# talmolab/VNL-Brax-Imitation

Hardware: AMD Instinct MI355X
Metric: env-steps/sec (whole node), rodent imitation, num_envs=4096/GPU (higher is better)
Workload: dtype f32; 1 GPU; rodent imitation rollout, single groom clip, 4096 envs/GPU: intention-policy forward (HIP) -> RodentTracking.step (5 substeps, CG 6/6) -> auto-reset on -> Transition logging (unroll 20, the 20 steps replayed as one captured hipGraph); envs_per_gpu=4096, clips=1, parallelism=env-sharded x1, no data-path collective

## Files before the change

### include/vnl.h

```cpp
#ifndef VNL_H_
#define VNL_H_

#include <stddef.h>
#include <stdint.h>

#ifdef __cplusplus
extern "C" {
#endif

#define VNL_OK 0
#define VNL_ERR_ARG -1
#define VNL_ERR_BLOB -2
#define VNL_ERR_HIP -3
#define VNL_ERR_NO_DEVICE -4
#define VNL_ERR_UNSUPPORTED -5

typedef struct vnl_model vnl_model;
typedef struct vnl_env vnl_env;
typedef struct vnl_policy vnl_policy;

typedef struct vnl_envspec {
  int32_t clip_frames;
  int32_t num_clips;
  int32_t ref_traj_length;
// ... 125 lines not shown
                       const float* rand_action ,
                       float* rand_log_prob ,
                       void* stream);

typedef struct vnl_policy_noise {
  uint64_t seed;
  const int64_t* step_base;
  int64_t step_offset;
  int64_t env_offset;
  float *eps_latent_out, *eps_action_out, *rand_action_out;
} vnl_policy_noise;
int vnl_policy_forward_noise(vnl_policy*, const float* params, const float* obs_mean, const float* obs_std,
                             const float* traj, const float* obs, const vnl_policy_noise*, int32_t batch,
                             int32_t deterministic, float* action, float* raw_action, float* log_prob, float* logits,
                             float* latent_mean, float* latent_logvar, float* rand_log_prob , void* stream);

#define VNL_POST_MAX_OPS 24
typedef struct vnl_post_op {
  float* dst;
  const float* src;
  const float* first;
  float* log;
  int32_t width;
  int32_t pad_;
} vnl_post_op;
typedef struct vnl_post_desc {
  float *steps, *prev_done, *done, *truncation;
  const float* reward;
  float *log_reward, *log_discount, *log_truncation;
  int32_t episode_length, action_repeat, num_ops, pad_;
  vnl_post_op ops[VNL_POST_MAX_OPS];
} vnl_post_desc;
int vnl_rollout_post(const vnl_post_desc*, int32_t num_envs, void* stream);

typedef struct vnl_ppo_head_args {
  int32_t T, B, act, latent;
  const float *logits, *baseline, *bootstrap, *lat_mean, *lat_logvar;
  const float *raw_action, *behaviour_log_prob, *reward, *truncation, *discount, *eps_entropy;
  float entropy_cost, discounting, reward_scaling, gae_lambda, clipping_epsilon, kl_weight, min_std, var_scale;
  int32_t normalize_advantage, pad_;
  float *g_logits, *g_baseline, *g_lat_mean, *g_lat_logvar;
  float *vs, *advantages;
  float *metrics;
} vnl_ppo_head_args;
#define VNL_PPO_HEAD_WORKSPACE_FLOATS (4 + 4 * 256)
int vnl_ppo_head(const vnl_ppo_head_args*, float* workspace, void* stream);

typedef struct vnl_gather_op {
  float* dst;
  const float* src;
  int32_t T, width;
} vnl_gather_op;
typedef struct vnl_gather_desc {
  const int64_t* idx;
  int32_t N, M, num_ops, pad_;
  vnl_gather_op ops[VNL_POST_MAX_OPS];
} vnl_gather_desc;
int vnl_gather_rows(const vnl_gather_desc*, void* stream);

int vnl_adam_step(float* params, const float* grads, float* mu, float* nu, const int64_t* count, int64_t n,
                  double lr, double b1, double b2, double eps, void* stream);

typedef struct vnl_ppo_net_spec {
  int32_t traj_size, obs_size, action_size, latent_size;
  int32_t num_encoder_layers, num_decoder_layers , num_value_layers ;
  int32_t encoder_layers[8], decoder_layers[8], value_layers[8];
// ... 38 lines not shown
```

### vnl-brax-imitation_amd/_lib.py

```python
from __future__ import annotations

import ctypes as C
import os

_HERE = os.path.dirname(os.path.abspath(__file__))
DEFAULT_LIB = os.path.join(_HERE, "csrc", "libvnl.so")

i32p = C.POINTER(C.c_int32)
f32p = C.POINTER(C.c_float)


class EnvSpec(C.Structure):
    _fields_ = [
        ("clip_frames", C.c_int32),
        ("num_clips", C.c_int32),
        ("ref_traj_length", C.c_int32),
        ("sub_clip_length", C.c_int32),
        ("n_frames", C.c_int32),
        ("num_track_bodies", C.c_int32),
        ("num_end_eff", C.c_int32),
        ("num_appendages", C.c_int32),
        ("num_joint_cols", C.c_int32),
        ("com_ref_col", C.c_int32),
        ("body_idxs", i32p),
# ... 106 lines not shown

PPO_HEAD_WORKSPACE_FLOATS = 4 + 4 * 256


class PPONetSpec(C.Structure):
    _fields_ = [(n, C.c_int32) for n in ("traj_size", "obs_size", "action_size", "latent_size", "num_encoder_layers",
                                          "num_decoder_layers", "num_value_layers")] + \
               [("encoder_layers", C.c_int32 * 8), ("decoder_layers", C.c_int32 * 8), ("value_layers", C.c_int32 * 8)]


class PPOBatch(C.Structure):
    _fields_ = [(n, C.c_void_p) for n in ("traj", "obs", "next_obs_last", "raw_action", "behaviour_log_prob", "reward",
                                          "truncation", "discount", "eps_latent", "eps_entropy", "obs_mean", "obs_std")]


class PPOHParams(C.Structure):
    _fields_ = [(n, C.c_float) for n in ("entropy_cost", "discounting", "reward_scaling", "gae_lambda",
                                         "clipping_epsilon", "kl_weight", "min_std", "var_scale")] + \
               [("normalize_advantage", C.c_int32), ("pad_", C.c_int32)]

class CorrPlan(C.Structure):
    _fields_ = [(n, C.c_int32) for n in ("route", "chunks", "chunk_cols", "row_tiles")] + [("workspace_floats", C.c_int64)]


class Domain(C.Structure):
    _fields_ = [(n, C.c_void_p) for n in ("cg_friction", "act_gain", "dof_damping", "dof_armature")]

class BodyDomain(C.Structure):
    _fields_ = [(n, C.c_void_p) for n in ("body_mass", "body_inertia", "body_ipos")]


EXPORTS = (
    "vnl_last_error", "vnl_version", "vnl_model_create", "vnl_model_destroy", "vnl_env_create", "vnl_env_destroy",
    "vnl_env_dims", "vnl_env_reset", "vnl_env_reset_done", "vnl_env_step", "vnl_env_fk", "vnl_env_debug", "vnl_env_scratch", "vnl_policy_create", "vnl_policy_destroy",
    "vnl_policy_num_params", "vnl_policy_forward", "vnl_policy_forward_noise", "vnl_rollout_post", "vnl_ppo_head", "vnl_adam_step", "vnl_gather_rows",
    "vnl_ppo_update_create", "vnl_ppo_update_destroy", "vnl_ppo_update_num_params", "vnl_ppo_update_buffer",
    "vnl_ppo_minibatch_grad",
    "vnl_ppo_minibatch_grad_part",
    "vnl_env_set_domain", "vnl_env_set_body_domain",
    "vnl_prediction_corr_plan", "vnl_prediction_corr",
)
_HIP_ONLY = ("vnl_policy_", "vnl_ppo_update_", "vnl_ppo_minibatch_", "vnl_prediction_corr")


class VnlError(RuntimeError):
    pass


def _declare(lib: C.CDLL) -> C.CDLL:
    vp = C.c_void_p
    lib.vnl_last_error.restype = C.c_char_p
    lib.vnl_version.restype = C.c_int
    lib.vnl_model_create.argtypes = [vp, C.c_size_t, C.POINTER(vp)]
    lib.vnl_model_destroy.argtypes = [vp]
    lib.vnl_model_destroy.restype = None
    lib.vnl_env_create.argtypes = [vp, C.POINTER(EnvSpec), C.c_int32, C.c_int32, C.POINTER(vp)]
    lib.vnl_env_destroy.argtypes = [vp]
    lib.vnl_env_destroy.restype = None
    lib.vnl_env_dims.argtypes = [vp, C.POINTER(Dims)]
    lib.vnl_env_reset.argtypes = [vp, vp, vp, C.POINTER(StatePtrs), vp]
    lib.vnl_env_reset_done.argtypes = [vp, vp, C.POINTER(ResetNoise), C.POINTER(StatePtrs), C.POINTER(ResetLog), C.c_int32, vp]
    lib.vnl_env_step.argtypes = [vp, vp, C.POINTER(StatePtrs), vp]
    lib.vnl_env_fk.argtypes = [vp, vp, C.POINTER(StatePtrs), vp]
    lib.vnl_env_debug.argtypes = [vp, C.c_int32, C.POINTER(C.c_int32)]
    lib.vnl_env_scratch.argtypes = [vp, C.c_char_p, C.POINTER(vp), C.POINTER(C.c_int32)]
    lib.vnl_env_set_domain.argtypes = [vp, C.POINTER(Domain), vp]
    lib.vnl_env_set_body_domain.argtypes = [vp, C.POINTER(BodyDomain), vp]
    lib.vnl_rollout_post.argtypes = [C.POINTER(PostDesc), C.c_int32, vp]
    lib.vnl_ppo_head.argtypes = [C.POINTER(PPOHeadArgs), vp, vp]
    lib.vnl_gather_rows.argtypes = [C.POINTER(GatherDesc), vp]
    lib.vnl_adam_step.argtypes = [vp, vp, vp, vp, vp, C.c_int64] + [C.c_double] * 4 + [vp]
    if hasattr(lib, "vnl_ppo_update_create"):
        lib.vnl_ppo_update_create.argtypes = [C.POINTER(PPONetSpec), C.c_int32, C.c_int32, C.c_int32, C.POINTER(vp)]
        lib.vnl_ppo_update_destroy.argtypes = [vp]
        lib.vnl_ppo_update_destroy.restype = None
        lib.vnl_ppo_update_num_params.argtypes = [vp]
        lib.vnl_ppo_update_num_params.restype = C.c_int64
        lib.vnl_ppo_update_buffer.argtypes = [vp, C.c_char_p, C.POINTER(vp), C.POINTER(C.c_int64)]
        lib.vnl_ppo_minibatch_grad.argtypes = [vp, vp, C.POINTER(PPOBatch), C.POINTER(PPOHParams), vp, vp, vp]
        lib.vnl_ppo_minibatch_grad_part.argtypes = [vp, vp, C.POINTER(PPOBatch), C.POINTER(PPOHParams), vp, vp, vp, C.c_int]
        lib.vnl_prediction_corr_plan.argtypes = [C.c_int32, C.c_int32, C.c_int32, C.POINTER(CorrPlan)]
        lib.vnl_prediction_corr.argtypes = [vp, vp, C.c_float, C.c_int32, C.c_int32, C.c_int32, vp, C.c_int64, vp, vp]
    if hasattr(lib, "vnl_policy_create"):
        lib.vnl_policy_create.argtypes = [C.POINTER(PolicySpec), C.c_int32, C.c_int32, C.POINTER(vp)]
        lib.vnl_policy_destroy.argtypes = [vp]
        lib.vnl_policy_destroy.restype = None
        lib.vnl_policy_num_params.argtypes = [vp]
        lib.vnl_policy_num_params.restype = C.c_int64
        lib.vnl_policy_forward.argtypes = [vp] + [vp] * 7 + [C.c_int32, C.c_int32] + [vp] * 6 + [vp, vp] + [vp]
        lib.vnl_policy_forward_noise.argtypes = [vp] + [vp] * 5 + [C.POINTER(PolicyNoise), C.c_int32, C.c_int32] + [vp] * 7 + [vp]
    return lib


_cache = {}

# ... 20 lines not shown
```

### vnl-brax-imitation_amd/csrc/vnl_domain.hip

```cpp
#include <hip/hip_runtime.h>
#include <stdint.h>

#include "../../include/vnl.h"
#ifdef VNL_PROFILE
#define g_vnl_prof g_vnl_prof_domain
#endif
#include "vnl_env_kernels.h"

int vnl_domain_reset_(const KernelConsts* kc, int spec, int B, size_t lds, void* stream, const DevState& ds, const int* start_frame,
                      const vreal* noise, vreal* dump, int* trace) {
  if (spec)
    hipLaunchKernelGGL((vnl_reset_kernel<VnlSpecDom<VnlSpecRodent>>), dim3(B), dim3(64), lds, (hipStream_t)stream, kc, ds,
                       start_frame, noise, dump, trace);
  else
    hipLaunchKernelGGL((vnl_reset_kernel<VnlSpecDom<VnlSpecGeneric>>), dim3(B), dim3(64), lds, (hipStream_t)stream, kc, ds,
                       start_frame, noise, dump, trace);
  return (int)hipGetLastError();
}

int vnl_domain_step_(const KernelConsts* kc, int spec, int B, size_t lds, void* stream, const DevState& ds, const vreal* action,
                     vreal* dump, vreal* dump_mid, int* trace) {
  if (spec)
    hipLaunchKernelGGL((vnl_step_kernel<VnlSpecDom<VnlSpecRodent>>), dim3(B), dim3(64), lds, (hipStream_t)stream, kc, ds,
                       action, dump, dump_mid, trace);
  else
    hipLaunchKernelGGL((vnl_step_kernel<VnlSpecDom<VnlSpecGeneric>>), dim3(B), dim3(64), lds, (hipStream_t)stream, kc, ds,
                       action, dump, dump_mid, trace);
  return (int)hipGetLastError();
}

int vnl_domain_reset_done_(const KernelConsts* kc, int spec, int B, size_t lds, void* stream, const DevState& ds,
                           const ResetDoneArgs& a, vreal* dump, int* trace) {
  if (spec)
    hipLaunchKernelGGL((vnl_reset_done_kernel<VnlSpecDom<VnlSpecRodent>>), dim3(B), dim3(64), lds, (hipStream_t)stream, kc, ds, a,
                       dump, trace);
  else
    hipLaunchKernelGGL((vnl_reset_done_kernel<VnlSpecDom<VnlSpecGeneric>>), dim3(B), dim3(64), lds, (hipStream_t)stream, kc, ds, a,
                       dump, trace);
  return (int)hipGetLastError();
}
```

### vnl-brax-imitation_amd/csrc/vnl_env_kernels.h

```cpp
#pragma once
#include "vnl_body.h"

#ifndef VNL_KERNEL_ATTR
#define VNL_KERNEL_ATTR
#endif
#define VNL_ENV_KERNEL __launch_bounds__(64) VNL_KERNEL_ATTR

template <class SP>
__global__ void VNL_ENV_KERNEL vnl_step_kernel(const KernelConsts* kc, DevState st, const vreal* action,
                                                      vreal* dump, vreal* dump_mid, int* trace) {
  VNL_LDS_DECL(lds);
  const VNL_CAS KernelConsts* k = VNL_TO_CAS(KernelConsts, kc);
  EnvWaveT<SP> w{k->m, k->ev, st, k->L, lds, blockIdx.x, threadIdx.x, k, nullptr};
  w.step(action, dump_mid, trace);
  if (dump) w.dump(dump);
}

template <class SP>
__global__ void VNL_ENV_KERNEL vnl_reset_kernel(const KernelConsts* kc, DevState st, const int* start_frame,
                                                       const vreal* noise, vreal* dump, int* trace) {
  VNL_LDS_DECL(lds);
  const VNL_CAS KernelConsts* k = VNL_TO_CAS(KernelConsts, kc);
  EnvWaveT<SP> w{k->m, k->ev, st, k->L, lds, blockIdx.x, threadIdx.x, k, nullptr};
  w.reset(start_frame, noise, trace);
  if (dump) w.dump(dump);
}


template <class SP>
__global__ void VNL_ENV_KERNEL vnl_reset_done_kernel(const KernelConsts* kc, DevState st, ResetDoneArgs a, vreal* dump, int* trace) {
  VNL_LDS_DECL(lds);
  const unsigned e = blockIdx.x, lane = threadIdx.x;
  if (a.mask[e] != 0.f) {
    const VNL_CAS KernelConsts* k = VNL_TO_CAS(KernelConsts, kc);
    EnvWaveT<SP> w{k->m, k->ev, st, k->L, lds, e, lane, k, nullptr};
    w.reset_fresh(a, trace);
    if (dump) w.dump(dump);
    VNL_SYNC_GLOBAL();
  }
  for (int q = 0; q < a.num_logs; q++) {
    const unsigned* src = a.logs[q].src + (size_t)e * a.logs[q].width;
    unsigned* log = a.logs[q].log + (size_t)e * a.logs[q].width;
    VNL_FOR(i, a.logs[q].width) log[i] = src[i];
  }
}
```

### vnl-brax-imitation_amd/csrc/vnl_lib.hip

```cpp
#include <hip/hip_runtime.h>
#include <stdint.h>
#include <stdio.h>
#include <stdlib.h>
#include <string.h>

#include <algorithm>
#include <cmath>
#include <cstddef>
#include <map>
#include <string>
#include <vector>

#include "../../include/vnl.h"
#include "vnl_body.h"

static thread_local char g_err[512] = "";
static int fail(int code, const char* fmt, const char* a = "", const char* b = "") {
  snprintf(g_err, sizeof(g_err), fmt, a, b);
  return code;
}
#define HIPCHK(call)                                                              \
  do {                                                                            \
    hipError_t e_ = (call);                                                       \
    if (e_ != hipSuccess) return fail(VNL_ERR_HIP, "%s: %s", #call, hipGetErrorString(e_)); \
// ... 958 lines not shown
  *count = it->second.second;
  return VNL_OK;
}

extern "C" int vnl_env_debug(vnl_env* env, int32_t enable, int32_t* row_stride) {
  if (!env) return fail(VNL_ERR_ARG, "vnl_env_debug: null argument");
  if (enable < 0 || enable > 2) return fail(VNL_ERR_ARG, "vnl_env_debug: mode must be 0, 1 or 2");
  if (enable && !env->dump) {
    void* p = nullptr;
    HIPCHK(hipMalloc(&p, (size_t)env->L.total * env->B * sizeof(vreal)));
    env->allocs.push_back(p);
    env->dump = (vreal*)p;
    const size_t nt = (size_t)env->B * (env->de.n_frames > 0 ? env->de.n_frames : 1) * VNL_TRACE_INTS * sizeof(int);
    HIPCHK(hipMalloc(&p, nt));
    env->allocs.push_back(p);
    HIPCHK(hipMemset(p, 0, nt));
    env->trace = (int*)p;
  }
  env->debug = enable;
  if (row_stride) *row_stride = env->L.total;
  return VNL_OK;
}

__global__ void __launch_bounds__(64) vnl_fk_kernel(const KernelConsts* kc, DevState st, const vreal* qpos) {
  VNL_LDS_DECL(lds);
  const VNL_CAS KernelConsts* k = VNL_TO_CAS(KernelConsts, kc);
  EnvWave w{k->m, k->ev, st, k->L, lds, blockIdx.x, threadIdx.x, k, nullptr};
  w.fk(qpos);
}

int vnl_domain_reset_(const KernelConsts* kc, int spec, int B, size_t lds, void* stream, const DevState& ds, const int* start_frame,
                      const vreal* noise, vreal* dump, int* trace);
int vnl_domain_step_(const KernelConsts* kc, int spec, int B, size_t lds, void* stream, const DevState& ds, const vreal* action,
                     vreal* dump, vreal* dump_mid, int* trace);
int vnl_domain_reset_done_(const KernelConsts* kc, int spec, int B, size_t lds, void* stream, const DevState& ds,
                           const ResetDoneArgs& a, vreal* dump, int* trace);

static int to_dev_state(const vnl_state* s, DevState* d) {
  const void* ptrs[] = {s->qpos, s->qvel, s->act, s->qacc_warmstart, s->xpos, s->xquat, s->subtree_com1,
                        s->qfrc_actuator, s->obs, s->reward, s->done, s->metrics, s->traj, s->termination_error,
                        s->cur_frame, s->sub_clip_frame, s->clip_id};
  for (const void* p : ptrs)
    if (!p) return fail(VNL_ERR_ARG, "vnl_state: null buffer");
  d->qpos = (vreal*)s->qpos, d->qvel = (vreal*)s->qvel, d->act = (vreal*)s->act, d->warm = (vreal*)s->qacc_warmstart;
  d->xpos = (vreal*)s->xpos, d->xquat = (vreal*)s->xquat, d->com1 = (vreal*)s->subtree_com1;
  d->qfrc_actuator = (vreal*)s->qfrc_actuator, d->obs = (vreal*)s->obs, d->reward = (vreal*)s->reward;
  d->done = (vreal*)s->done, d->metrics = (vreal*)s->metrics, d->traj = (vreal*)s->traj;
  d->term_err = (vreal*)s->termination_error, d->cur_frame = s->cur_frame, d->sub_clip_frame = s->sub_clip_frame;
  d->clip_id = s->clip_id;
  return VNL_OK;
}

extern "C" int vnl_env_reset(vnl_env* env, const int32_t* start_frame, const float* noise, const vnl_state* state,
                             void* stream) {
  if (!env || !start_frame || !noise || !state) return fail(VNL_ERR_ARG, "vnl_env_reset: null argument");
  DevState ds;
  int rc = to_dev_state(state, &ds);
  if (rc != VNL_OK) return rc;
  DeviceGuard guard(env->device);
  if (!guard.ok) return fail(VNL_ERR_HIP, "hipSetDevice failed");
  if (env->has_dom) {
    HIPCHK((hipError_t)vnl_domain_reset_(env->kc, env->spec, env->B, env->lds_bytes, stream, ds, (const int*)start_frame,
                                         (const vreal*)noise, env->debug ? env->dump : nullptr, env->debug ? env->trace : nullptr));
    return VNL_OK;
  }
  if (env->spec)
    hipLaunchKernelGGL((vnl_reset_kernel<VnlSpecRodent>), dim3(env->B), dim3(64), env->lds_bytes, (hipStream_t)stream,
// ... 33 lines not shown
  for (int k = 0; k < num_logs; k++)
    a.logs[k].src = (const unsigned*)logs[k].src, a.logs[k].log = (unsigned*)logs[k].log, a.logs[k].width = logs[k].width;
  DeviceGuard guard(env->device);
  if (!guard.ok) return fail(VNL_ERR_HIP, "hipSetDevice failed");
  vreal* dump = env->debug ? env->dump : nullptr;
  int* trace = env->debug ? env->trace : nullptr;
  if (env->has_dom) {
    HIPCHK((hipError_t)vnl_domain_reset_done_(env->kc, env->spec, env->B, env->lds_bytes, stream, ds, a, dump, trace));
    return VNL_OK;
  }
  if (env->spec)
    hipLaunchKernelGGL((vnl_reset_done_kernel<VnlSpecRodent>), dim3(env->B), dim3(64), env->lds_bytes, (hipStream_t)stream,
                       (const KernelConsts*)env->kc, ds, a, dump, trace);
  else
    hipLaunchKernelGGL((vnl_reset_done_kernel<VnlSpecGeneric>), dim3(env->B), dim3(64), env->lds_bytes, (hipStream_t)stream,
                       (const KernelConsts*)env->kc, ds, a, dump, trace);
  HIPCHK(hipGetLastError());
  return VNL_OK;
}

extern "C" int vnl_env_fk(vnl_env* env, const float* qpos, const vnl_state* state, void* stream) {
  if (!env || !qpos || !state) return fail(VNL_ERR_ARG, "vnl_env_fk: null argument");
  DevState ds;
  int rc = to_dev_state(state, &ds);
  if (rc != VNL_OK) return rc;
  DeviceGuard guard(env->device);
  if (!guard.ok) return fail(VNL_ERR_HIP, "hipSetDevice failed");
  hipLaunchKernelGGL(vnl_fk_kernel, dim3(env->B), dim3(64), env->lds_bytes, (hipStream_t)stream, (const KernelConsts*)env->kc, ds,
                     (const vreal*)qpos);
  HIPCHK(hipGetLastError());
  return VNL_OK;
}

extern "C" int vnl_env_step(vnl_env* env, const float* action, const vnl_state* state, void* stream) {
  if (!env || !action || !state) return fail(VNL_ERR_ARG, "vnl_env_step: null argument");
  DevState ds;
  int rc = to_dev_state(state, &ds);
  if (rc != VNL_OK) return rc;
  DeviceGuard guard(env->device);
  if (!guard.ok) return fail(VNL_ERR_HIP, "hipSetDevice failed");
  if (env->has_dom) {
    HIPCHK((hipError_t)vnl_domain_step_(env->kc, env->spec, env->B, env->lds_bytes, stream, ds, (const vreal*)action,
                                        env->debug == 1 ? env->dump : nullptr, env->debug == 2 ? env->dump : nullptr,
                                        env->debug ? env->trace : nullptr));
    return VNL_OK;
  }
  if (env->spec)
    hipLaunchKernelGGL((vnl_step_kernel<VnlSpecRodent>), dim3(env->B), dim3(64), env->lds_bytes, (hipStream_t)stream,
                       (const KernelConsts*)env->kc, ds, (const vreal*)action, env->debug == 1 ? env->dump : nullptr,
                       env->debug == 2 ? env->dump : nullptr, env->debug ? env->trace : nullptr);
  else
    hipLaunchKernelGGL((vnl_step_kernel<VnlSpecGeneric>), dim3(env->B), dim3(64), env->lds_bytes, (hipStream_t)stream,
                       (const KernelConsts*)env->kc, ds, (const vreal*)action, env->debug == 1 ? env->dump : nullptr,
                       env->debug == 2 ? env->dump : nullptr, env->debug ? env->trace : nullptr);
  HIPCHK(hipGetLastError());
  return VNL_OK;
}


static std::vector<vreal> four_field_tables(const vnl_env* env, const std::vector<double> v[4]) {
  const DevModel& d = env->dm;
  std::vector<vreal> tab;
  tab.reserve((size_t)env->B * (2 * d.ncg + d.nu + 2 * d.nv));
  for (double x : v[0]) tab.push_back((vreal)x);
  for (size_t k = 0; k < v[0].size(); k++) tab.push_back((vreal)contact_invweight(env->cg_t[k % d.ncg], v[0][k], env->impratio));
  for (int f = 1; f < 4; f++)
    for (double x : v[f]) tab.push_back((vreal)x);
  return tab;
}
static std::vector<vreal> four_field_compiled(const vnl_env* env) {
  const std::vector<double>* model[4] = {&env->mu0, &env->gain0, &env->damp0, &env->arm0};
  std::vector<double> v[4];
  for (int f = 0; f < 4; f++)
    for (int e = 0; e < env->B; e++) v[f].insert(v[f].end(), model[f]->begin(), model[f]->end());
  return four_field_tables(env, v);
}

static const char* body_row(const vnl_env* env, const double* mass, const double* inertia, const double* ipos, std::vector<double>* out,
                            char* why, size_t nwhy) {
  const int nb = env->fmap->nb_out, nd = env->dm.nbody;
  std::vector<double> full;
  if (inertia) {
    full = env->ifull0;
    for (int b = 1; b < nb; b++) {
      double dl[3], R[9];
      for (int k = 0; k < 3; k++) dl[k] = inertia[3 * (size_t)b + k] - env->inertia0[3 * (size_t)b + k];
      if (dl[0] == 0 && dl[1] == 0 && dl[2] == 0) continue;
      qmat_d(&env->iquat0[4 * (size_t)b], R);
      for (int r = 0; r < 3; r++)
// ... 207 lines not shown
  const unsigned e = blockIdx.x, tid = threadIdx.x;
  float st = d.steps ? ((d.prev_done && d.prev_done[e] != 0.f) ? 0.f : d.steps[e]) + (float)d.action_repeat : 0.f;
  float done = d.done[e];
  bool over = d.steps && st >= (float)d.episode_length;
  float trunc = over ? 1.f - done : 0.f;
  done = over ? 1.f : done;
  __syncthreads();
  if (tid == 0) {
    if (d.steps) d.steps[e] = st;
    if (d.prev_done) d.prev_done[e] = done;
    d.done[e] = done;
    if (d.truncation) d.truncation[e] = trunc;
    if (d.log_reward) d.log_reward[e] = d.reward[e];
    if (d.log_discount) d.log_discount[e] = 1.f - done;
    if (d.log_truncation) d.log_truncation[e] = trunc;
  }
  const bool reset = done != 0.f;
  for (int k = 0; k < d.num_ops; k++) {
    const vnl_post_op& op = d.ops[k];
    const bool from_first = op.first && reset;
    const unsigned* src = (const unsigned*)(from_first ? op.first : op.src) + (size_t)e * op.width;
    unsigned* dst = op.dst ? (unsigned*)op.dst + (size_t)e * op.width : nullptr;
    unsigned* log = op.log ? (unsigned*)op.log + (size_t)e * op.width : nullptr;
    const bool store = dst && (from_first || (const float*)op.dst != op.src);
    for (int i = (int)tid; i < op.width; i += VNL_POST_THREADS) {
      unsigned v = src[i];
      if (store) dst[i] = v;
      if (log) log[i] = v;
    }
  }
}

extern "C" int vnl_rollout_post(const vnl_post_desc* desc, int32_t num_envs, void* stream) {
  if (!desc || num_envs <= 0 || !desc->done) return fail(VNL_ERR_ARG, "vnl_rollout_post: null argument");
  if (desc->num_ops < 0 || desc->num_ops > VNL_POST_MAX_OPS) return fail(VNL_ERR_ARG, "vnl_rollout_post: too many ops");
  for (int k = 0; k < desc->num_ops; k++)
    if (!desc->ops[k].src || desc->ops[k].width <= 0) return fail(VNL_ERR_ARG, "vnl_rollout_post: bad op");
  if ((desc->log_reward && !desc->reward)) return fail(VNL_ERR_ARG, "vnl_rollout_post: log_reward without reward");
  hipLaunchKernelGGL(vnl_post_kernel, dim3(num_envs), dim3(VNL_POST_THREADS), 0, (hipStream_t)stream, *desc);
  HIPCHK(hipGetLastError());
  return VNL_OK;
}

#ifndef VNL_HEAD_THREADS
#define VNL_HEAD_THREADS 256
#define VNL_HEAD_GROUP 32
#define VNL_GROUP_SUM(v) \
  (v += __shfl_xor(v, 16, 32), v += __shfl_xor(v, 8, 32), v += __shfl_xor(v, 4, 32), v += __shfl_xor(v, 2, 32), v += __shfl_xor(v, 1, 32))
#endif
#define VNL_HEAD_MAXBLK 256
#ifndef VNL_FINISH_THREADS
#define VNL_FINISH_THREADS 64
#define VNL_FINISH_SUM(v) \
  (v += __shfl_xor(v, 32), v += __shfl_xor(v, 16), v += __shfl_xor(v, 8), v += __shfl_xor(v, 4), v += __shfl_xor(v, 2), v += __shfl_xor(v, 1))
#endif
__device__ __forceinline__ float vnl_block_sum(float v, float* red) {
  const unsigned tid = threadIdx.x;
  __syncthreads();
  red[tid] = v;
  __syncthreads();
  for (unsigned w = VNL_HEAD_THREADS / 2; w > 0; w >>= 1) {
    if (tid < w) red[tid] += red[tid + w];
    __syncthreads();
  }
  return red[0];
}
__device__ __forceinline__ float vnl_softplus(float x) { return x > 20.f ? x : log1pf(expf(x)); }

__global__ void __launch_bounds__(VNL_HEAD_THREADS) vnl_ppo_gae_kernel(vnl_ppo_head_args a, float* stats) {
#if VNL_HEAD_THREADS > 1
  __shared__ float red[VNL_HEAD_THREADS];
// ... 226 lines not shown
```

### vnl-brax-imitation_amd/envs/rodent.py

```python
from __future__ import annotations

import ctypes as C
import os
from typing import Any, Dict, List, Mapping, Optional, Sequence

import numpy as np
import torch

from .. import _lib
from ..model import blob as _blob
from ..model import mjcf as _mjcf
from .base import Env, PipelineState, State

_PKG = os.path.dirname(os.path.dirname(os.path.abspath(__file__)))
_TEST_BACKEND = None
_METRICS = ("rcom", "rvel", "rtrunk", "rquat", "ract", "rapp", "termination_error")
DOMAIN_FIELDS = {"cg_friction": ("ngeom_collide", 0.0, False), "act_gain": ("nu", None, False),
                 "dof_damping": ("nv", 0.0, True), "dof_armature": ("nv", 0.0, True)}
BODY_DOMAIN_FIELDS = {"body_mass": ((), 0.0), "body_inertia": ((3,), 0.0), "body_ipos": ((3,), None)}


def packaged_model_path(name: str = "rodent", scale_factor: Optional[float] = 0.9) -> str:
    if scale_factor is None:
        return os.path.join(_PKG, "data", f"{name}.npz")
# ... 335 lines not shown
        nz.start_hi = self._start_hi()
        nz.noise_scale = self._reset_noise_scale
        record = record or {}
        for k, dt in (("start_frame", torch.int32), ("clip_id", torch.int32), ("noise", self._dtype)):
            t = record.get(k)
            if t is not None:
                if t.dtype != dt or not t.is_contiguous() or t.shape[0] != B or t.device != self.device:
                    raise ValueError(f"record[{k!r}] must be a contiguous {dt} tensor with {B} rows on the env's device")
                setattr(nz, k + "_out", t.data_ptr())
        logs = tuple(logs)
        if len(logs) > _lib.RESET_MAX_LOGS:
            raise ValueError(f"at most {_lib.RESET_MAX_LOGS} logs")
        arr = (_lib.ResetLog * max(len(logs), 1))()
        for o, (src, log) in zip(arr, logs):
            if src.dtype not in (torch.float32, torch.int32) or log.dtype != src.dtype or src.shape != log.shape or \
                    src.shape[0] != B or not (src.is_contiguous() and log.is_contiguous()):
                raise ValueError("a log is a (src, log) pair of contiguous float32 / int32 tensors of one shape (B[, w])")
            o.src, o.log, o.width = src.data_ptr(), log.data_ptr(), src.numel() // B
        p = self._ptrs(state)
        _lib.check(self._L, self._L.vnl_env_reset_done(self._env_h, mk.data_ptr(), C.byref(nz), C.byref(p), arr, len(logs),
                                                       self._stream()))
        self._hold = (mk, step_base, logs, record)
        return state

    def step(self, state: State, action: torch.Tensor) -> State:
        nu, B = int(self.dims.nu), self.num_envs
        if tuple(action.shape) != (B, nu):
            raise ValueError(f"action must be ({B},{nu}), got {tuple(action.shape)}")
        a = action.to(device=self.device, dtype=self._dtype).contiguous()
        p = self._ptrs(state)
        ev = getattr(self, "kernel_events", None)
        if ev is not None:
            ev[0].record()
        _lib.check(self._L, self._L.vnl_env_step(self._env_h, a.data_ptr(), C.byref(p), self._stream()))
        if ev is not None:
            ev[1].record()
        self._hold = (a,)
        return state

    def forward_kinematics(self, qpos: torch.Tensor, out: Optional[State] = None) -> State:
        B, nq = self.num_envs, int(self.dims.nq)
        if tuple(qpos.shape) != (B, nq):
            raise ValueError(f"qpos must be ({B},{nq}), got {tuple(qpos.shape)}")
        state = out if out is not None else self._alloc_state()
        q = qpos.to(device=self.device, dtype=self._dtype).contiguous()
        state.pipeline_state.qpos.copy_(q)
        p = self._ptrs(state)
        _lib.check(self._L, self._L.vnl_env_fk(self._env_h, q.data_ptr(), C.byref(p), self._stream()))
        self._hold = (q,)
        return state

    def debug(self, mode=True) -> None:
        stride = C.c_int32()
        _lib.check(self._L, self._L.vnl_env_debug(self._env_h, int(mode), C.byref(stride)))
        self._dump_stride = stride.value

    def solver_trace(self) -> torch.Tensor:
        ptr, cnt = C.c_void_p(), C.c_int32()
        _lib.check(self._L, self._L.vnl_env_scratch(self._env_h, b"solver_trace", C.byref(ptr), C.byref(cnt)))
        B, n = self.num_envs, cnt.value
        if self.device.type == "cuda":
            torch.cuda.synchronize(self.device)
            flat = torch.empty(B * n, dtype=torch.int32, device=self.device)
            rc = C.CDLL("libamdhip64.so").hipMemcpy(C.c_void_p(flat.data_ptr()), ptr, C.c_size_t(4 * B * n), C.c_int(3))
            if rc != 0:
                raise _lib.VnlError(f"hipMemcpy failed: {rc}")
            flat = flat.cpu()
# ... 27 lines not shown
```

### vnl-brax-imitation_amd/ppo_imitation/acting.py

```python
from __future__ import annotations

import dataclasses
import time
from typing import Any, Callable, Dict, Optional, Sequence, Tuple

import numpy as np
import torch

from ..envs.base import State
from ..envs.wrappers import EvalWrapper


@dataclasses.dataclass
class Transition:

    observation: torch.Tensor
    action: torch.Tensor
    reward: torch.Tensor
    discount: torch.Tensor
    next_observation: torch.Tensor
    extras: Dict[str, Dict[str, torch.Tensor]]

    def map(self, fn: Callable[[torch.Tensor], torch.Tensor]) -> "Transition":
        return Transition(fn(self.observation), fn(self.action), fn(self.reward), fn(self.discount),
                          fn(self.next_observation),
                          {k: {kk: fn(vv) for kk, vv in v.items()} for k, v in self.extras.items()})


def actor_step(env, env_state: State, policy, key, extra_fields: Sequence[str] = ()) -> Tuple[State, Transition]:
    obs = env_state.obs.clone()
    traj = env_state.info["traj"]
    actions, policy_extras = policy(traj, obs, key)
    nstate = env.step(env_state, actions)
    state_extras = {x: nstate.info[x] for x in extra_fields}
    return nstate, Transition(observation=obs, action=actions, reward=nstate.reward, discount=1 - nstate.done,
                              next_observation=nstate.obs,
                              extras={"policy_extras": policy_extras, "state_extras": state_extras})


def _fusable(env):
    from ..envs import wrappers as W

    if not isinstance(env, W.AutoResetWrapper) or not isinstance(env.env, W.EpisodeWrapper):
        return None
    ep, base = env.env, env.env.env
    if ep.action_repeat != 1 or base is not base.unwrapped or not hasattr(getattr(base, "_L", None), "vnl_rollout_post"):
        return None
    return env, ep, base


def _device_noise(policy) -> bool:
    return getattr(policy, "noise", None) == "device"


_DIRECT_LOG = True


def _generate_unroll_fused(fz, env_state: State, policy, key, unroll_length: int, extra_fields) -> Tuple[State, Transition]:
    import ctypes as C

    from .. import _lib

    ar, ep, base = fz
    st = env_state
    T, info, dev = unroll_length, env_state.info, env_state.obs.device
    B = st.obs.shape[0]
    new = lambda *shape, like: torch.empty((T, *shape), dtype=like.dtype, device=dev)
    obs0, nobs_log = st.obs.clone(), new(*st.obs.shape, like=st.obs)
    rew_log, disc_log = new(B, like=st.reward), new(B, like=st.reward)
    sx_log = {x: new(*info[x].shape, like=info[x]) for x in extra_fields}
    prev_done = st.done.clone()
    stream = C.c_void_p(torch.cuda.current_stream(dev).cuda_stream) if dev.type == "cuda" else C.c_void_p(0)
    ptr = lambda t: C.c_void_p(t.data_ptr()) if t is not None else C.c_void_p(0)
    width = lambda t: 1 if t.dim() == 1 else t.shape[1]

    d = _lib.PostDesc()
    d.steps, d.prev_done, d.done, d.truncation, d.reward = (ptr(info["steps"]), ptr(prev_done), ptr(st.done),
                                                            ptr(info["truncation"]), ptr(st.reward))
    d.episode_length, d.action_repeat = ep.episode_length, 1
    ops = []
    fresh = getattr(ar, "mode", "first_state") == "fresh"
    if fresh:
        reset_logs = [(st.obs, nobs_log)] + [(info[x], sx_log[x]) for x in extra_fields if x != "truncation"]
    else:
        fps = info["first_pipeline_state"]
        for name in st.pipeline_state._FIELDS:
            cur = st.pipeline_state.raw(name)
            ops.append((cur, cur, fps.raw(name), None))
        ops.append((st.obs, st.obs, info["first_obs"], nobs_log))
        logged = set()
        if ar.reset_info:
            for k2, v in info["first_info"].items():
                ops.append((info[k2], info[k2], v, sx_log.get(k2)))
                logged.add(k2)
        for x in extra_fields:
            if x not in logged and x != "truncation":
                ops.append((None, info[x], None, sx_log[x]))
    n_static = len(ops)
    px_log: Optional[dict] = None
    act_log = None
    dev_noise = _device_noise(policy)
    direct = dev_noise and _DIRECT_LOG
    if direct:
        na = base.action_size
        f32 = lambda *shape: torch.empty((T, *shape), dtype=torch.float32, device=dev)
        act_log = f32(B, na)
        px_log = {} if policy.deterministic else {"log_prob": f32(B), "rand_log_prob": f32(B), "raw_action": f32(B, na),
                                                  "logits": f32(B, 2 * na)}
    for t in range(T):
        if direct:
            actions, pex = policy(info["traj"], st.obs, None, step_offset=t, advance=False,
                                  out={"action": act_log[t], **{k2: v[t] for k2, v in px_log.items()}})
        elif dev_noise:
            actions, pex = policy(info["traj"], st.obs, None, step_offset=t, advance=False)
        else:
            actions, pex = policy(info["traj"], st.obs, key)
        base.step(st, actions)
        if px_log is None:
            act_log = new(*actions.shape, like=actions)
            px_log = {k2: new(*v.shape, like=v) for k2, v in pex.items()}
        step_ops = ops[:n_static] if direct else ops[:n_static] + [(None, actions.contiguous(), None, act_log)] + \
            [(None, v.contiguous(), None, px_log[k2]) for k2, v in pex.items()]
        assert len(step_ops) <= _lib.POST_MAX_OPS
        d.num_ops = len(step_ops)
        keep = []
        for i, (dst, src, first, log) in enumerate(step_ops):
            assert src.dtype in (torch.float32, torch.int32) and src.is_contiguous()
            o = d.ops[i]
            o.dst, o.src, o.first, o.width = ptr(dst), ptr(src), ptr(first), width(src)
            o.log = ptr(log[t]) if log is not None else C.c_void_p(0)
            keep.append(src)
        d.log_reward, d.log_discount = ptr(rew_log[t]), ptr(disc_log[t])
        d.log_truncation = ptr(sx_log["truncation"][t]) if "truncation" in sx_log else C.c_void_p(0)
        _lib.check(base._L, base._L.vnl_rollout_post(C.byref(d), B, stream))
        _generate_unroll_fused.hold = keep
        if fresh:
            base.reset_done(st, st.done, seed=ar.seed, step_base=info["reset_step"], step_offset=t, env_offset=ar.env_offset,
                            logs=[(src, log[t]) for src, log in reset_logs])
    if fresh:
        info["reset_step"].add_(T)
    if dev_noise:
        policy.counter.add_(T)
    obs_log = torch.cat((obs0[None], nobs_log[:-1]), dim=0)
    data = Transition(observation=obs_log, action=act_log, reward=rew_log, discount=disc_log, next_observation=nobs_log,
                      extras={"policy_extras": px_log, "state_extras": sx_log})
    return st, data


class GraphedUnroll:

    def __init__(self, env, env_state: State, policy, key: torch.Generator, unroll_length: int,
                 extra_fields: Sequence[str] = ()):
        fz = _fusable(env)
        dev = env_state.obs.device
        if fz is None or dev.type != "cuda":
            raise ValueError("GraphedUnroll needs AutoResetWrapper(EpisodeWrapper(<env on a HIP device>)), action_repeat 1")
        dev_noise = _device_noise(policy)
        if not dev_noise and (key is None or key.device.type != "cuda"):
            raise ValueError("GraphedUnroll needs a torch.Generator on the device (its stream is captured with the graph)")
        self._args = (fz, env_state, policy, key, int(unroll_length), tuple(extra_fields))
        self.state = env_state
        gen_state = policy.counter.clone() if dev_noise else key.get_state()
        saved = _snapshot_state(env_state)
        side = torch.cuda.Stream(dev)
        side.wait_stream(torch.cuda.current_stream(dev))
        with torch.cuda.stream(side):
            _generate_unroll_fused(*self._args)
# ... 99 lines not shown
```

Before: 2.665 million env-steps/s.

## Fuse rollout post-processing into env step kernel as an epilogue

The separate vnl_rollout_post kernel, which handles step counting, truncation, done flags and transition logging copies, now runs as an epilogue at the end of the env step kernel when a post descriptor is supplied. The unroll loop passes the descriptor to RodentTracking.step, which calls the new vnl_env_step_post entry point. This removes one kernel launch per step from the captured graph. In exchange, the copies run on only 64 lanes per env inside the heavy step kernel, which has its own occupancy limits, and the large descriptor passed by value may add register or kernarg pressure.

```diff
diff --git a/include/vnl.h b/include/vnl.h
--- a/include/vnl.h
+++ b/include/vnl.h
@@ -181,6 +181,7 @@
   vnl_post_op ops[VNL_POST_MAX_OPS];
 } vnl_post_desc;
 int vnl_rollout_post(const vnl_post_desc*, int32_t num_envs, void* stream);
+int vnl_env_step_post(vnl_env*, const float* action, const vnl_state* state, const vnl_post_desc* desc, void* stream);
 
 typedef struct vnl_ppo_head_args {
   int32_t T, B, act, latent;
diff --git a/vnl-brax-imitation_amd/_lib.py b/vnl-brax-imitation_amd/_lib.py
--- a/vnl-brax-imitation_amd/_lib.py
+++ b/vnl-brax-imitation_amd/_lib.py
@@ -162,7 +162,7 @@
 
 EXPORTS = (
     "vnl_last_error", "vnl_version", "vnl_model_create", "vnl_model_destroy", "vnl_env_create", "vnl_env_destroy",
-    "vnl_env_dims", "vnl_env_reset", "vnl_env_reset_done", "vnl_env_step", "vnl_env_fk", "vnl_env_debug", "vnl_env_scratch", "vnl_policy_create", "vnl_policy_destroy",
+    "vnl_env_dims", "vnl_env_reset", "vnl_env_reset_done", "vnl_env_step", "vnl_env_step_post", "vnl_env_fk", "vnl_env_debug", "vnl_env_scratch", "vnl_policy_create", "vnl_policy_destroy",
     "vnl_policy_num_params", "vnl_policy_forward", "vnl_policy_forward_noise", "vnl_rollout_post", "vnl_ppo_head", "vnl_adam_step", "vnl_gather_rows",
     "vnl_ppo_update_create", "vnl_ppo_update_destroy", "vnl_ppo_update_num_params", "vnl_ppo_update_buffer",
     "vnl_ppo_minibatch_grad",
@@ -191,6 +191,8 @@
     lib.vnl_env_reset.argtypes = [vp, vp, vp, C.POINTER(StatePtrs), vp]
     lib.vnl_env_reset_done.argtypes = [vp, vp, C.POINTER(ResetNoise), C.POINTER(StatePtrs), C.POINTER(ResetLog), C.c_int32, vp]
     lib.vnl_env_step.argtypes = [vp, vp, C.POINTER(StatePtrs), vp]
+    if hasattr(lib, "vnl_env_step_post"):
+        lib.vnl_env_step_post.argtypes = [vp, vp, C.POINTER(StatePtrs), C.POINTER(PostDesc), vp]
     lib.vnl_env_fk.argtypes = [vp, vp, C.POINTER(StatePtrs), vp]
     lib.vnl_env_debug.argtypes = [vp, C.c_int32, C.POINTER(C.c_int32)]
     lib.vnl_env_scratch.argtypes = [vp, C.c_char_p, C.POINTER(vp), C.POINTER(C.c_int32)]
diff --git a/vnl-brax-imitation_amd/csrc/vnl_domain.hip b/vnl-brax-imitation_amd/csrc/vnl_domain.hip
--- a/vnl-brax-imitation_amd/csrc/vnl_domain.hip
+++ b/vnl-brax-imitation_amd/csrc/vnl_domain.hip
@@ -19,13 +19,13 @@
 }
 
 int vnl_domain_step_(const KernelConsts* kc, int spec, int B, size_t lds, void* stream, const DevState& ds, const vreal* action,
-                     vreal* dump, vreal* dump_mid, int* trace) {
+                     vreal* dump, vreal* dump_mid, int* trace, const vnl_post_desc& post) {
   if (spec)
     hipLaunchKernelGGL((vnl_step_kernel<VnlSpecDom<VnlSpecRodent>>), dim3(B), dim3(64), lds, (hipStream_t)stream, kc, ds,
-                       action, dump, dump_mid, trace);
+                       action, dump, dump_mid, trace, post);
   else
     hipLaunchKernelGGL((vnl_step_kernel<VnlSpecDom<VnlSpecGeneric>>), dim3(B), dim3(64), lds, (hipStream_t)stream, kc, ds,
-                       action, dump, dump_mid, trace);
+                       action, dump, dump_mid, trace, post);
   return (int)hipGetLastError();
 }
 
diff --git a/vnl-brax-imitation_amd/csrc/vnl_env_kernels.h b/vnl-brax-imitation_amd/csrc/vnl_env_kernels.h
--- a/vnl-brax-imitation_amd/csrc/vnl_env_kernels.h
+++ b/vnl-brax-imitation_amd/csrc/vnl_env_kernels.h
@@ -1,4 +1,5 @@
 #pragma once
+#include "../../include/vnl.h"
 #include "vnl_body.h"
 
 #ifndef VNL_KERNEL_ATTR
@@ -6,14 +7,84 @@
 #endif
 #define VNL_ENV_KERNEL __launch_bounds__(64) VNL_KERNEL_ATTR
 
+#define VNL_POST_BATCH 16
+#ifdef VNL_FORKJOIN_DEFINED
+#define VNL_POST_LANDED(x)
+#else
+#define VNL_POST_LANDED(x) asm volatile("" : "+v"(x))
+#endif
+VNL_HD void vnl_post_epilogue(const vnl_post_desc& d, const unsigned e, const unsigned lane) {
+  VNL_SYNC_GLOBAL();
+  const float old_prev = (d.prev_done ? d.prev_done : d.done)[e], old_steps = (d.steps ? d.steps : d.done)[e];
+  const float rew = (d.reward ? d.reward : d.done)[e];
+  float done = d.done[e];
+  float st = d.steps ? ((d.prev_done && old_prev != 0.f) ? 0.f : old_steps) + (float)d.action_repeat : 0.f;
+  bool over = d.steps && st >= (float)d.episode_length;
+  float trunc = over ? 1.f - done : 0.f;
+  done = over ? 1.f : done;
+  VNL_SYNC_GLOBAL();
+  VNL_SERIAL {
+    if (d.steps) d.steps[e] = st;
+    if (d.prev_done) d.prev_done[e] = done;
+    d.done[e] = done;
+    if (d.truncation) d.truncation[e] = trunc;
+    if (d.log_reward) d.log_reward[e] = rew;
+    if (d.log_discount) d.log_discount[e] = 1.f - done;
+    if (d.log_truncation) d.log_truncation[e] = trunc;
+  }
+  const bool reset = done != 0.f;
+  const int n = d.num_ops;
+  int k = 0, base = 0;
+  const unsigned* src = nullptr;
+  unsigned *dst = nullptr, *log = nullptr;
+  int width = 0;
+  while (k < n) {
+    unsigned v[VNL_POST_BATCH];
+    unsigned *pd[VNL_POST_BATCH], *pl[VNL_POST_BATCH];
+#pragma unroll
+    for (int j = 0; j < VNL_POST_BATCH; j++) {
+      pd[j] = pl[j] = nullptr;
+      v[j] = 0u;
+      if (k < n) {
+        if (base == 0) {
+          const float *o_src = d.ops[k].src, *o_first = d.ops[k].first;
+          float *o_dst = d.ops[k].dst, *o_log = d.ops[k].log;
+          width = d.ops[k].width;
+          const bool from_first = o_first && reset;
+          const size_t row = (size_t)e * width;
+          src = (const unsigned*)(from_first ? o_first : o_src) + row;
+          dst = (o_dst && (from_first || (const float*)o_dst != o_src)) ? (unsigned*)o_dst + row : nullptr;
+          log = o_log ? (unsigned*)o_log + row : nullptr;
+        }
+        const int i = base + (int)lane;
+        if (i < width) {
+          v[j] = src[i];
+          pd[j] = dst ? dst + i : nullptr;
+          pl[j] = log ? log + i : nullptr;
+        }
+        base += VNL_LANES;
+        if (base >= width) k++, base = 0;
+      }
+    }
+#pragma unroll
+    for (int j = 0; j < VNL_POST_BATCH; j++) VNL_POST_LANDED(v[j]);
+#pragma unroll
+    for (int j = 0; j < VNL_POST_BATCH; j++) {
+      if (pd[j]) *pd[j] = v[j];
+      if (pl[j]) *pl[j] = v[j];
+    }
+  }
+}
+
 template <class SP>
 __global__ void VNL_ENV_KERNEL vnl_step_kernel(const KernelConsts* kc, DevState st, const vreal* action,
-                                                      vreal* dump, vreal* dump_mid, int* trace) {
+                                                      vreal* dump, vreal* dump_mid, int* trace, vnl_post_desc post) {
   VNL_LDS_DECL(lds);
   const VNL_CAS KernelConsts* k = VNL_TO_CAS(KernelConsts, kc);
   EnvWaveT<SP> w{k->m, k->ev, st, k->L, lds, blockIdx.x, threadIdx.x, k, nullptr};
   w.step(action, dump_mid, trace);
   if (dump) w.dump(dump);
+  if (post.num_ops >= 0) vnl_post_epilogue(post, blockIdx.x, threadIdx.x);
 }
 
 template <class SP>
diff --git a/vnl-brax-imitation_amd/csrc/vnl_lib.hip b/vnl-brax-imitation_amd/csrc/vnl_lib.hip
--- a/vnl-brax-imitation_amd/csrc/vnl_lib.hip
+++ b/vnl-brax-imitation_amd/csrc/vnl_lib.hip
@@ -1014,7 +1014,7 @@
 int vnl_domain_reset_(const KernelConsts* kc, int spec, int B, size_t lds, void* stream, const DevState& ds, const int* start_frame,
                       const vreal* noise, vreal* dump, int* trace);
 int vnl_domain_step_(const KernelConsts* kc, int spec, int B, size_t lds, void* stream, const DevState& ds, const vreal* action,
-                     vreal* dump, vreal* dump_mid, int* trace);
+                     vreal* dump, vreal* dump_mid, int* trace, const vnl_post_desc& post);
 int vnl_domain_reset_done_(const KernelConsts* kc, int spec, int B, size_t lds, void* stream, const DevState& ds,
                            const ResetDoneArgs& a, vreal* dump, int* trace);
 
@@ -1114,29 +1114,53 @@
   return VNL_OK;
 }
 
-extern "C" int vnl_env_step(vnl_env* env, const float* action, const vnl_state* state, void* stream) {
-  if (!env || !action || !state) return fail(VNL_ERR_ARG, "vnl_env_step: null argument");
+static int post_desc_check(const vnl_post_desc* desc, int32_t num_envs) {
+  if (!desc || num_envs <= 0 || !desc->done) return fail(VNL_ERR_ARG, "vnl_rollout_post: null argument");
+  if (desc->num_ops < 0 || desc->num_ops > VNL_POST_MAX_OPS) return fail(VNL_ERR_ARG, "vnl_rollout_post: too many ops");
+  for (int k = 0; k < desc->num_ops; k++)
+    if (!desc->ops[k].src || desc->ops[k].width <= 0) return fail(VNL_ERR_ARG, "vnl_rollout_post: bad op");
+  if ((desc->log_reward && !desc->reward)) return fail(VNL_ERR_ARG, "vnl_rollout_post: log_reward without reward");
+  return VNL_OK;
+}
+
+static int env_step_launch(vnl_env* env, const float* action, const vnl_state* state, const vnl_post_desc* post, void* stream) {
   DevState ds;
   int rc = to_dev_state(state, &ds);
   if (rc != VNL_OK) return rc;
   DeviceGuard guard(env->device);
   if (!guard.ok) return fail(VNL_ERR_HIP, "hipSetDevice failed");
+  vnl_post_desc none{};
+  none.num_ops = -1;
+  const vnl_post_desc& pd = post ? *post : none;
   if (env->has_dom) {
     HIPCHK((hipError_t)vnl_domain_step_(env->kc, env->spec, env->B, env->lds_bytes, stream, ds, (const vreal*)action,
                                         env->debug == 1 ? env->dump : nullptr, env->debug == 2 ? env->dump : nullptr,
-                                        env->debug ? env->trace : nullptr));
+                                        env->debug ? env->trace : nullptr, pd));
     return VNL_OK;
   }
   if (env->spec)
     hipLaunchKernelGGL((vnl_step_kernel<VnlSpecRodent>), dim3(env->B), dim3(64), env->lds_bytes, (hipStream_t)stream,
                        (const KernelConsts*)env->kc, ds, (const vreal*)action, env->debug == 1 ? env->dump : nullptr,
-                       env->debug == 2 ? env->dump : nullptr, env->debug ? env->trace : nullptr);
+                       env->debug == 2 ? env->dump : nullptr, env->debug ? env->trace : nullptr, pd);
   else
     hipLaunchKernelGGL((vnl_step_kernel<VnlSpecGeneric>), dim3(env->B), dim3(64), env->lds_bytes, (hipStream_t)stream,
                        (const KernelConsts*)env->kc, ds, (const vreal*)action, env->debug == 1 ? env->dump : nullptr,
-                       env->debug == 2 ? env->dump : nullptr, env->debug ? env->trace : nullptr);
+                       env->debug == 2 ? env->dump : nullptr, env->debug ? env->trace : nullptr, pd);
   HIPCHK(hipGetLastError());
   return VNL_OK;
+}
+
+extern "C" int vnl_env_step(vnl_env* env, const float* action, const vnl_state* state, void* stream) {
+  if (!env || !action || !state) return fail(VNL_ERR_ARG, "vnl_env_step: null argument");
+  return env_step_launch(env, action, state, nullptr, stream);
+}
+
+extern "C" int vnl_env_step_post(vnl_env* env, const float* action, const vnl_state* state, const vnl_post_desc* desc,
+                                 void* stream) {
+  if (!env || !action || !state) return fail(VNL_ERR_ARG, "vnl_env_step_post: null argument");
+  int rc = post_desc_check(desc, env->B);
+  if (rc != VNL_OK) return rc;
+  return env_step_launch(env, action, state, desc, stream);
 }
 
 
@@ -1410,11 +1434,8 @@
 }
 
 extern "C" int vnl_rollout_post(const vnl_post_desc* desc, int32_t num_envs, void* stream) {
-  if (!desc || num_envs <= 0 || !desc->done) return fail(VNL_ERR_ARG, "vnl_rollout_post: null argument");
-  if (desc->num_ops < 0 || desc->num_ops > VNL_POST_MAX_OPS) return fail(VNL_ERR_ARG, "vnl_rollout_post: too many ops");
-  for (int k = 0; k < desc->num_ops; k++)
-    if (!desc->ops[k].src || desc->ops[k].width <= 0) return fail(VNL_ERR_ARG, "vnl_rollout_post: bad op");
-  if ((desc->log_reward && !desc->reward)) return fail(VNL_ERR_ARG, "vnl_rollout_post: log_reward without reward");
+  int rc = post_desc_check(desc, num_envs);
+  if (rc != VNL_OK) return rc;
   hipLaunchKernelGGL(vnl_post_kernel, dim3(num_envs), dim3(VNL_POST_THREADS), 0, (hipStream_t)stream, *desc);
   HIPCHK(hipGetLastError());
   return VNL_OK;
diff --git a/vnl-brax-imitation_amd/envs/rodent.py b/vnl-brax-imitation_amd/envs/rodent.py
--- a/vnl-brax-imitation_amd/envs/rodent.py
+++ b/vnl-brax-imitation_amd/envs/rodent.py
@@ -391,7 +391,11 @@
         ev = getattr(self, "kernel_events", None)
         if ev is not None:
             ev[0].record()
-        _lib.check(self._L, self._L.vnl_env_step(self._env_h, a.data_ptr(), C.byref(p), self._stream()))
+        post, self._post_desc = getattr(self, "_post_desc", None), None
+        if post is not None:
+            _lib.check(self._L, self._L.vnl_env_step_post(self._env_h, a.data_ptr(), C.byref(p), C.byref(post), self._stream()))
+        else:
+            _lib.check(self._L, self._L.vnl_env_step(self._env_h, a.data_ptr(), C.byref(p), self._stream()))
         if ev is not None:
             ev[1].record()
         self._hold = (a,)
diff --git a/vnl-brax-imitation_amd/ppo_imitation/acting.py b/vnl-brax-imitation_amd/ppo_imitation/acting.py
--- a/vnl-brax-imitation_amd/ppo_imitation/acting.py
+++ b/vnl-brax-imitation_amd/ppo_imitation/acting.py
@@ -54,6 +54,7 @@
 
 
 _DIRECT_LOG = True
+_POST_EPILOGUE = True
 
 
 def _generate_unroll_fused(fz, env_state: State, policy, key, unroll_length: int, extra_fields) -> Tuple[State, Transition]:
@@ -101,6 +102,8 @@
     act_log = None
     dev_noise = _device_noise(policy)
     direct = dev_noise and _DIRECT_LOG
+    from ..envs.rodent import RodentTracking
+    epilogue = _POST_EPILOGUE and hasattr(base._L, "vnl_env_step_post") and type(base).step is RodentTracking.step
     if direct:
         na = base.action_size
         f32 = lambda *shape: torch.empty((T, *shape), dtype=torch.float32, device=dev)
@@ -115,7 +118,8 @@
             actions, pex = policy(info["traj"], st.obs, None, step_offset=t, advance=False)
         else:
             actions, pex = policy(info["traj"], st.obs, key)
-        base.step(st, actions)
+        if not epilogue:
+            base.step(st, actions)
         if px_log is None:
             act_log = new(*actions.shape, like=actions)
             px_log = {k2: new(*v.shape, like=v) for k2, v in pex.items()}
@@ -132,7 +136,14 @@
             keep.append(src)
         d.log_reward, d.log_discount = ptr(rew_log[t]), ptr(disc_log[t])
         d.log_truncation = ptr(sx_log["truncation"][t]) if "truncation" in sx_log else C.c_void_p(0)
-        _lib.check(base._L, base._L.vnl_rollout_post(C.byref(d), B, stream))
+        if epilogue:
+            base._post_desc = d
+            try:
+                base.step(st, actions)
+            finally:
+                base._post_desc = None
+        else:
+            _lib.check(base._L, base._L.vnl_rollout_post(C.byref(d), B, stream))
         _generate_unroll_fused.hold = keep
         if fresh:
             base.reset_done(st, st.done, seed=ar.seed, step_base=info["reset_step"], step_offset=t, env_offset=ar.env_offset,
```

Measured after the change: 2.713 million env-steps/s (median of 6 runs). 1.8% higher.
